# mindspore-lab/minddiffusion

Measured on AMD Instinct MI355X. Metric: 512x512 txt2img latents/sec (50-step DDIM), higher is better.
Workload: dtype f16; 1 GPU; SDv2 txt2img 512x512 (64x64 latent), 50-step DDIM, CFG 9.0, batch 1 per GPU (BASELINE.json configs[1]); synthetic seeded weights + synthetic text conditioning; global_batch=1, parallelism=batch-shard x1, hip_graph=True, rccl_world_size=1, broadcast_bytes=0, ddim_steps=50, unet_batch_per_gpu=2, sampler=ddim, cfg_dup_prefix=False

## Files before the change

include/mdx.h:

```cpp
#ifndef MDX_H_
#define MDX_H_

#include <stddef.h>
#include <stdint.h>

#ifdef __cplusplus
extern "C" {
#endif

#define MDX_OK 0
#define MDX_E_INVALID (-1)
#define MDX_E_WORKSPACE (-2)
#define MDX_E_HIP (-3)

typedef void* mdx_stream_t;

int mdx_version(void);
const char* mdx_last_error(void);
int mdx_set_option(const char* name, int value);
int mdx_get_option(const char* name, int* value);

int mdx_nchw_to_nhwc_f16(const float* x, void* y, int B, int C, int H, int W, int Cpad, mdx_stream_t s);
int mdx_nhwc_to_nchw_f32(const void* x, float* y, int B, int C, int H, int W, int Cstride, mdx_stream_t s);

// ... 77 lines not shown
    float xattn_scale;
    const float* act_slope;
    int act_slope_n;
    int geglu_unit;
} mdx_gemm_desc;

#define MDX_GEMM_WS_HEAD 16384
#define MDX_EPI_NONE 0
#define MDX_EPI_GEGLU 1
#define MDX_EPI_GELU 2
#define MDX_EPI_QUICKGELU 3
#define MDX_EPI_PRELU 4
#define MDX_OUT_ROWMAJOR 0
#define MDX_OUT_TRANSPOSED 1
#define MDX_OUT_D2S2 2

int mdx_gemm_f16(const mdx_gemm_desc* d, mdx_stream_t s);
int mdx_gemm_release_counters(void);
int mdx_gemm_release_workspace(const void* workspace);
int mdx_gemm_bind_counters(const void* workspace, void* counters);
size_t mdx_gemm_workspace_bytes(const mdx_gemm_desc* d);
int mdx_gemm_check(const mdx_gemm_desc* d);
int mdx_gemm_query(const mdx_gemm_desc* d, int* out7);
int mdx_gemm_tune(const mdx_gemm_desc* d, mdx_stream_t s, void* flush, size_t flush_bytes, int reps, int* best4, float* us2);

int mdx_groupnorm_from_splitk_f16(const mdx_gemm_desc* prod, const float* gamma, const float* beta, void* y, int groups,
                                  float eps, int silu, mdx_stream_t s);
int mdx_groupnorm_from_splitk_ok(const mdx_gemm_desc* prod, int groups);

int mdx_attention_f16(const void* q, long q_bs, int q_ld, const void* k, long k_bs, int k_ld, const void* vt,
                      long vt_bs, int vt_ld, void* o, long o_bs, int o_ld, int B, int heads, int D, int Nq, int Nk,
                      float scale, mdx_stream_t s);

size_t mdx_attention_ws_bytes(int B, int heads, int D, int Nq, int Nk);
int mdx_attention_splitkv_f16(const void* q, long q_bs, int q_ld, const void* k, long k_bs, int k_ld, const void* vt,
                              long vt_bs, int vt_ld, void* o, long o_bs, int o_ld, int B, int heads, int D, int Nq, int Nk,
                              float scale, int kv_splits, void* ws, size_t ws_bytes, mdx_stream_t s);

typedef struct mdx_st_tail_desc {
    const void* attn_out;
    const void* tok;
    const void* x_in;
    void* out;
    const void* ctx_k;
    const void* ctx_vt;
    const void* wstream;
// ... 141 lines not shown
```

minddiffusion_amd/_lib.py:

```python
import ctypes
import os

_HERE = os.path.dirname(os.path.abspath(__file__))
LIB_PATH = os.environ.get("MDX_LIBRARY") or os.path.join(_HERE, "libmdx.so")

c_void_p = ctypes.c_void_p
c_int = ctypes.c_int
c_long = ctypes.c_long
c_float = ctypes.c_float
c_size_t = ctypes.c_size_t


class MdxError(RuntimeError):
    pass


class GemmDesc(ctypes.Structure):
    _fields_ = [
        ("a", c_void_p), ("a2", c_void_p), ("c1", c_int), ("c2", c_int),
        ("w", c_void_p), ("bias", c_void_p), ("rowbias", c_void_p), ("rowbias_ld", c_int),
        ("residual", c_void_p), ("residual_ld", c_int),
        ("out", c_void_p), ("out_ld", c_int),
        ("B", c_int), ("H", c_int), ("W", c_int), ("N", c_int),
        ("ksize", c_int), ("stride", c_int), ("upsample", c_int),
# ... 58 lines not shown
                                  c_int, c_float, c_int, c_void_p, c_void_p]),
    "mdx_groupnorm_query": (c_int, [c_int, c_int, c_int, c_int, c_int, c_int, ctypes.POINTER(c_int)]),
    "mdx_groupnorm_colstats_f16": (c_int, [c_void_p, c_int, c_void_p, c_int, c_void_p, c_int, c_void_p, c_int, c_void_p,
                                           c_void_p, c_void_p, c_void_p, c_int, c_void_p, c_int, c_int, c_int, c_float,
                                           c_int, c_void_p]),
    "mdx_colstats_fold_f32": (c_int, [c_void_p, c_int, c_void_p, c_int, c_int, c_int, c_void_p]),
    "mdx_groupnorm_from_splitk_f16": (c_int, [ctypes.POINTER(GemmDesc), c_void_p, c_void_p, c_void_p, c_int, c_float, c_int,
                                              c_void_p]),
    "mdx_groupnorm_from_splitk_ok": (c_int, [ctypes.POINTER(GemmDesc), c_int]),
    "mdx_groupnorm_scaleshift_f16": (c_int, [c_void_p, c_int, c_void_p, c_int, c_void_p, c_void_p, c_void_p, c_void_p,
                                             c_int, c_void_p, c_int, c_int, c_int, c_float, c_int, c_void_p, c_void_p]),
    "mdx_layernorm_f16": (c_int, [c_void_p, c_void_p, c_void_p, c_void_p, c_int, c_int, c_float, c_void_p]),
    "mdx_gemm_f16": (c_int, [ctypes.POINTER(GemmDesc), c_void_p]),
    "mdx_gemm_workspace_bytes": (c_size_t, [ctypes.POINTER(GemmDesc)]),
    "mdx_gemm_release_workspace": (c_int, [c_void_p]),
    "mdx_gemm_bind_counters": (c_int, [c_void_p, c_void_p]),
    "mdx_st_tail_sched_barriers": (c_int, [c_int, c_int]),
    "mdx_st_head_sched_barriers": (c_int, [c_int, c_int]),
    "mdx_gemm_release_counters": (c_int, []),
    "mdx_gemm_tune": (c_int, [ctypes.POINTER(GemmDesc), c_void_p, c_void_p, c_size_t, c_int, ctypes.POINTER(c_int),
                              ctypes.POINTER(ctypes.c_float)]),
    "mdx_gemm_check": (c_int, [ctypes.POINTER(GemmDesc)]),
    "mdx_gemm_query": (c_int, [ctypes.POINTER(GemmDesc), ctypes.POINTER(c_int)]),
    "mdx_attention_f16": (c_int, [c_void_p, c_long, c_int, c_void_p, c_long, c_int, c_void_p, c_long, c_int,
                                  c_void_p, c_long, c_int, c_int, c_int, c_int, c_int, c_int, c_float, c_void_p]),
    "mdx_attention_ws_bytes": (c_size_t, [c_int, c_int, c_int, c_int, c_int]),
    "mdx_attention_splitkv_f16": (c_int, [c_void_p, c_long, c_int, c_void_p, c_long, c_int, c_void_p, c_long, c_int,
                                          c_void_p, c_long, c_int, c_int, c_int, c_int, c_int, c_int, c_float, c_int, c_void_p,
                                          c_size_t, c_void_p]),
    "mdx_attention_causal_f16": (c_int, [c_void_p, c_long, c_int, c_void_p, c_long, c_int, c_void_p, c_long, c_int,
                                  c_void_p, c_long, c_int, c_int, c_int, c_int, c_int, c_int, c_float, c_void_p]),
    "mdx_st_head_f16": (c_int, [ctypes.POINTER(StHeadDesc), c_void_p]),
    "mdx_st_head_supported": (c_int, [c_int, c_int, c_int]),
    "mdx_st_head_stream_bytes": (c_size_t, [c_int]),
    "mdx_st_tail_f16": (c_int, [ctypes.POINTER(StTailDesc), c_void_p]),
    "mdx_st_tail_supported": (c_int, [c_int, c_int, c_int, c_int, c_int]),
    "mdx_st_tail_stream_bytes": (c_size_t, [c_int]),
    "mdx_lora_merge_f16": (c_int, [ctypes.POINTER(LoraMergeDesc), c_void_p]),
    "mdx_timestep_embedding_f32": (c_int, [c_void_p, c_void_p, c_int, c_int, c_float, c_void_p]),
    "mdx_dense_small_f32": (c_int, [c_void_p, c_int, c_void_p, c_void_p, c_void_p, c_int, c_int, c_int, c_int,
                                    c_int, c_int, c_void_p]),
    "mdx_sampler_step_f32": (c_int, [c_void_p, c_void_p, c_void_p, c_int, c_float, c_void_p, c_void_p, c_void_p,
                                     c_void_p, c_float, c_float, c_float, c_float, c_float, c_void_p, c_void_p,
                                     c_void_p, c_void_p, c_int, c_int, c_int, c_int, c_void_p]),
    "mdx_sampler_step_pred_f32": (c_int, [c_void_p, c_void_p, c_void_p, c_void_p, c_int, c_float, c_int, c_float, c_float,
                                          c_void_p, c_void_p, c_void_p, c_void_p, c_float, c_float, c_float, c_float,
# ... 77 lines not shown
```

minddiffusion_amd/csrc/gemm.hip:

```cpp
#include "mdx_common.h"
#include "gemm_internal.h"

#include <algorithm>
#include <type_traits>

namespace {


template <int BM, int BN, int BK, int NS, bool SWAP, bool FASTK, int NW, bool GNA = false, bool EXT = false>
__global__ __launch_bounds__(NW * 64, NW == 4 ? 2 : 1) void gemm_kernel(const GemmParams p) {
    mdx_kernarg_touch<sizeof(GemmParams)>();
    constexpr int WROWS = BM / (NW / 2);
    constexpr int TM = WROWS / 32;
    constexpr int TN = BN / 64;
    static_assert(TM >= 1, "tile too short for this many waves");
    constexpr int ROWB = BK * 2;
    constexpr int CPRW = BK / 8;
    constexpr int RPI = 64 / CPRW;
    constexpr int RP256 = 256 / ROWB;
    constexpr int KS = BK / 16;
    constexpr int A_BYTES = BM * ROWB;
    constexpr int B_BYTES = BN * ROWB;
    constexpr int STAGE = A_BYTES + B_BYTES;
    constexpr int AJ = BM / RPI / NW;
// ... 314 lines not shown
                rdfrag(I1{}, ks + 1);
                __builtin_amdgcn_sched_barrier(0);
                mfmas(I0{});
                __builtin_amdgcn_sched_barrier(0);
                if (ks + 2 < KS) {
                    rdfrag(I0{}, ks + 2);
                    __builtin_amdgcn_sched_barrier(0);
                }
                mfmas(I1{});
                __builtin_amdgcn_sched_barrier(0);
            }
        }
        rd = (rd + 1 == NS) ? 0 : rd + 1;
        wr = (wr + 1 == NS) ? 0 : wr + 1;
    }

    __syncthreads();
    trace_mark(p, 3);
    if constexpr (SWAP) asm volatile("" ::"v"(touch_ln), "v"(touch_s));
    gemm_epilogue<BM, BN, SWAP, NW, LinearRows, 0, 0, EXT>(p, acc, smem, LinearRows{m0}, n0, split, bpre, tile_m, tile_id);
    trace_mark(p, 4);
}

template <int BM, int BN, int NSB, bool SWAP, int PW, bool BDIR = false, bool W4 = false>
__global__ __launch_bounds__(BM * 2, BM == 128 ? 2 : 1) void conv3x3_halo_kernel(const GemmParams p) {
    static_assert(PW == 16 || (PW == 8 && BM == 128), "patch width 16, or 8 with two-sample tiles");
    static_assert(!W4 || (BDIR && BM == 128 && BN == 128 && !SWAP), "W4: weight-streaming 128 x 128 tiles with slab output");
    constexpr int NW = BM / 32;
    constexpr int PH = BM / 16;
    constexpr int HWD = PW + 2;
    constexpr int WROWS = W4 ? BM : BM / (NW / 2);
    constexpr int TM = WROWS / 32;
    constexpr int TN = W4 ? 1 : BN / 64;
    constexpr int HROWS = PW == 16 ? (PH + 2) * 18 : (BM / 64) * 100;
    constexpr int HINST = (HROWS + 7) / 8;
    constexpr int HALO_BYTES = HINST * 1024;
    constexpr int HJ = (HINST + NW - 1) / NW;
    constexpr int B_BYTES = BN * 128;
    constexpr int BJ = BN / 8 / NW;
    static_assert(BJ >= 1, "weight tile too small for this many loader waves");
    extern __shared__ __attribute__((aligned(16))) char smem[];
    mdx_kernarg_touch<sizeof(GemmParams)>();

    const int tid = threadIdx.x;
    const int lane = tid & 63;
    const int wave = __builtin_amdgcn_readfirstlane(tid >> 6);
    const int wm = W4 ? 0 : wave >> 1, wn = W4 ? wave : wave & 1;
    const int hi = lane >> 5;
    const int l31 = lane & 31;
// ... 159 lines not shown
                for (int r = 0; r < 16; ++r) {
                    const int row = i * 32 + (r & 3) + 8 * (r >> 2) + 4 * hi;
                    int m;
                    if constexpr (PW == 16)
                        m = (pb * p.H + py0) * p.W + px0 + (row >> 4) * p.W + (row & 15);
                    else
                        m = tile_m * BM + row;
                    if (m < p.M && n < p.N) wsz[(size_t)m * p.N + n] = acc[i][0][r];
                }
            trace_mark(p, 4);
            return;
        } else {
            if constexpr (PW == 16)
                gemm_epilogue<BM, BN, SWAP, NW, PatchRows, 0, 2>(p, acc, smem, PatchRows{(pb * p.H + py0) * p.W + px0, p.W, pb}, n0,
                                                                          split, bpre, tile_m, tile_id);
            else
                gemm_epilogue<BM, BN, SWAP, NW>(p, acc, smem, LinearRows{tile_m * BM}, n0, split, bpre, tile_m, tile_id);
            trace_mark(p, 4);
            return;
        }
    }
    if constexpr (!BDIR) {
    float2* gn_tab = reinterpret_cast<float2*>(smem + 2 * HALO_BYTES + NSB * B_BYTES);
    if constexpr (PW == 16) {
        if (p.gn_cs) {
            float2* csum = reinterpret_cast<float2*>(smem);
            const int cpg = p.cin >> 5;
            const float2* src = reinterpret_cast<const float2*>(p.gn_cs) + (size_t)pb * p.gn_nrb * p.cin;
            for (int c = tid; c < p.cin; c += NW * 64) {
                float su = 0.f, sq = 0.f;
                int k = 0;
                for (; k + 8 <= p.gn_nrb; k += 8) {
                    float2 v[8];
#pragma unroll
                    for (int e = 0; e < 8; ++e) v[e] = src[(size_t)(k + e) * p.cin + c];
#pragma unroll
                    for (int e = 0; e < 8; ++e) {
                        su += v[e].x;
                        sq += v[e].y;
                    }
                }
                for (; k < p.gn_nrb; ++k) {
                    const float2 v = src[(size_t)k * p.cin + c];
                    su += v.x;
                    sq += v.y;
                }
                csum[c] = make_float2(su, sq);
// ... 14 lines not shown
                const float a = p.gn_gamma[c] * rsqrtf(var + p.gn_eps);
                gn_tab[c] = make_float2(a, p.gn_beta[c] - mean * a);
            }
            __syncthreads();
        }
    }
    auto gn_transform = [&](int chunk, int hb) {
#pragma unroll
        for (int q = 0; q < HJ; ++q) {
            if (wave * HJ + q >= HINST || hal_off[q] == MDX_OOB) continue;
            char* pc = smem + hb * HALO_BYTES + (wave * HJ + q) * 1024 + lane * 16;
            const int ch0 = chunk * 64 + (int)((hal_off[q] >> 4) & 7u) * 8;
            const f16x8 x = *reinterpret_cast<const f16x8*>(pc);
            f16x8 y;
#pragma unroll
            for (int e = 0; e < 8; ++e) {
                const float2 t = gn_tab[ch0 + e];
                const float v = (float)x[e] * t.x + t.y;
                y[e] = (f16)(p.gn_silu ? silu_f(v) : v);
            }
            *reinterpret_cast<f16x8*>(pc) = y;
        }
    };
#pragma unroll
    for (int q = 0; q < HJ; ++q) dma_halo(q, c_begin, 0);
#pragma unroll
    for (int i = 0; i < NSB - 1; ++i)
        if (i < nt) dma_b(kt_begin + i, i);

    int t = 0;
    int rd = 0, wr = NSB - 1;
    trace_mark(p, 1);
    for (int c = c_begin; c < c_end; ++c) {
        const int hb = (c - c_begin) & 1;
        const bool more = c + 1 < c_end;
#pragma unroll
        for (int tap = 0; tap < 9; ++tap, ++t) {
            if (NSB >= 4 && t + 2 < nt)
                asm volatile("s_waitcnt vmcnt(%0)" ::"n"(2 * BJ) : "memory");
            else if (NSB >= 3 && t + 1 < nt)
                asm volatile("s_waitcnt vmcnt(%0)" ::"n"(BJ) : "memory");
            else
                asm volatile("s_waitcnt vmcnt(0)" ::: "memory");
            if constexpr (PW == 16) {
                if (tap == 0 && p.gn_cs) {
                    gn_transform(c, hb);
// ... 50 lines not shown
                rdfrag(I0{}, 0); rdfrag(I1{}, 1); rdfrag(I2{}, 2); rdfrag(I3{}, 3);
                __builtin_amdgcn_sched_barrier(0);
                mfmas(I0{}); mfmas(I1{}); mfmas(I2{}); mfmas(I3{});
            } else {
                rdfrag(I0{}, 0);
                __builtin_amdgcn_sched_barrier(0);
#pragma unroll
                for (int ks = 0; ks < 4; ks += 2) {
                    rdfrag(I1{}, ks + 1);
                    __builtin_amdgcn_sched_barrier(0);
                    mfmas(I0{});
                    __builtin_amdgcn_sched_barrier(0);
                    if (ks + 2 < 4) {
                        rdfrag(I0{}, ks + 2);
                        __builtin_amdgcn_sched_barrier(0);
                    }
                    mfmas(I1{});
                    __builtin_amdgcn_sched_barrier(0);
                }
            }
            rd = (rd + 1 == NSB) ? 0 : rd + 1;
            wr = (wr + 1 == NSB) ? 0 : wr + 1;
        }
    }

    if (p.skip_w) {
        constexpr int SA_BYTES = BM * 128;
        static_assert(2 * SA_BYTES <= 2 * HALO_BYTES && NSB >= 2, "skip tiles reuse the halo / ring areas");
        const __amdgpu_buffer_rsrc_t rs_s1 = make_rsrc(p.skip_a, p.skip_a_bytes);
        const __amdgpu_buffer_rsrc_t rs_s2 = make_rsrc(p.skip_a2 ? p.skip_a2 : p.skip_a, p.skip_a2 ? p.skip_a2_bytes : p.skip_a_bytes);
        const __amdgpu_buffer_rsrc_t rs_sw = make_rsrc(p.skip_w, p.skip_w_bytes);
        const int sk_begin = split * p.skip_kt_per_split, sk_end = min(p.skip_kt, sk_begin + p.skip_kt_per_split);
        constexpr int SAJ = BM / 8 / NW;
        int s_pix[SAJ];
        unsigned s_cb[SAJ];
#pragma unroll
        for (int j = 0; j < SAJ; ++j) {
            const int row = (wave * SAJ + j) * 8 + lrow;
            int pix;
            if constexpr (PW == 16) {
                pix = (pb * p.H + py0 + (row >> 4)) * p.W + px0 + (row & 15);
            } else {
                pix = tile_m * BM + row;
                if (pix >= p.M) pix = -1;
            }
            s_pix[j] = pix;
// ... 304 lines not shown
            launch_one<BM, BN, BK, NS, false, false, NW>(p, grid, st);
    }
}

template <int BM, int BN>
bool launch_bn(const GemmParams& p, int ns, bool swap, bool fastk, dim3 grid, hipStream_t st, bool nw8 = false) {
    if constexpr (BM == 128) {
        if (nw8 && (ns == 2 || ns == 3)) {
            if (ns == 2) launch_cfg<128, BN, 64, 2, 8>(p, swap, fastk, grid, st); else launch_cfg<128, BN, 64, 3, 8>(p, swap, fastk, grid, st);
            return true;
        }
    }
    if (ns == 2) launch_cfg<BM, BN, 64, 2, 4>(p, swap, fastk, grid, st);
    else if (ns == 3) launch_cfg<BM, BN, 64, 3, 4>(p, swap, fastk, grid, st);
    else if (BM == 128 && ns == 4) launch_cfg<128, BN, 64, 4, 4>(p, swap, fastk, grid, st);
    else if (BM == 128 && ns == 5) launch_cfg<128, BN, 64, 5, 4>(p, swap, fastk, grid, st);
    else if (BM == 64 && ns == 4) launch_cfg<64, BN, 64, 4, 4>(p, swap, fastk, grid, st);
    else if (BM == 64 && ns == 5) launch_cfg<64, BN, 64, 5, 4>(p, swap, fastk, grid, st);
    else if (BM == 64 && ns == 6) launch_cfg<64, BN, 64, 6, 4>(p, swap, fastk, grid, st);
    else return false;
    return true;
}

template <int BM, int BN, int NSB, bool SWAP, int PW = 16, bool BDIR = false, bool W4 = false>
void launch_halo(const GemmParams& p, dim3 grid, hipStream_t st) {
    constexpr size_t hinst = ((PW == 16 ? (BM / 16 + 2) * 18 : (BM / 64) * 100) + 7) / 8;
    constexpr size_t ring = 2 * hinst * 1024 + (BDIR ? 0 : (size_t)NSB * BN * 128);
    constexpr size_t epi = (size_t)BM * (BN + 8) * 2 + 4096;
    constexpr size_t lds0 = ring > epi ? ring : epi;
    constexpr size_t gn_tab_max = (BDIR || PW != 16) ? 0 : 640 * 8;
    const size_t lds = lds0 + (p.gn_cs ? (size_t)p.cin * 8 : 0);
    static MdxPerDeviceOnce attr_once;
    if (attr_once.first()) {
        (void)hipFuncSetAttribute(reinterpret_cast<const void*>(&conv3x3_halo_kernel<BM, BN, NSB, SWAP, PW, BDIR, W4>),
                                  hipFuncAttributeMaxDynamicSharedMemorySize, (int)(lds0 + gn_tab_max));
    }
    hipLaunchKernelGGL((conv3x3_halo_kernel<BM, BN, NSB, SWAP, PW, BDIR, W4>), grid, dim3(BM * 2), lds, st, p);
}

template <int BN, int PW>
void launch_halo_bdir(const GemmParams& p, bool swap, dim3 grid, hipStream_t st) {
    if (swap) launch_halo<128, BN, 2, true, PW, true>(p, grid, st); else launch_halo<128, BN, 2, false, PW, true>(p, grid, st);
}
template <int PW>
void launch_halo_bdir_w4(const GemmParams& p, dim3 grid, hipStream_t st) {
    launch_halo<128, 128, 2, false, PW, true, true>(p, grid, st);
}

template <int BM, int BN, int PW = 16>
void launch_halo_cfg(const GemmParams& p, int nsb, bool swap, dim3 grid, hipStream_t st) {
    if (nsb == 4) {
        if (swap) launch_halo<BM, BN, 4, true, PW>(p, grid, st); else launch_halo<BM, BN, 4, false, PW>(p, grid, st);
    } else if (nsb == 3) {
        if (swap) launch_halo<BM, BN, 3, true, PW>(p, grid, st); else launch_halo<BM, BN, 3, false, PW>(p, grid, st);
    } else {
        if (swap) launch_halo<BM, BN, 2, true, PW>(p, grid, st); else launch_halo<BM, BN, 2, false, PW>(p, grid, st);
    }
}

}

int mdx_gemm_launch_plan(const GemmParams& p, const GemmPlan& pl, hipStream_t st) {
    const dim3 grid = pl.grid;
    const bool swap = pl.swap, wide = pl.bn == 128;
    int rc;
    switch (pl.form) {
        case GEMM_CONV8P:
            rc = mdx_conv8p_launch(p, pl.bn, st);
            if (rc != MDX_OK) return rc;
            MDX_LAUNCH_CHECK("mdx_gemm_f16(conv8p)");
            return MDX_OK;
        case GEMM_LEAN:
        case GEMM_LEAN_XA:
            rc = mdx_dense_launch(p, pl, st);
            if (rc != MDX_OK) return rc;
            break;
        case GEMM_HALO:
            if (pl.bm == 256) {
                if (wide) launch_halo_cfg<256, 128>(p, pl.ring, swap, grid, st); else launch_halo_cfg<256, 64>(p, pl.ring, swap, grid, st);
            } else if (pl.pw == 8) {
                if (wide) launch_halo_cfg<128, 128, 8>(p, pl.ring, swap, grid, st); else launch_halo_cfg<128, 64, 8>(p, pl.ring, swap, grid, st);
            } else {
                if (wide) launch_halo_cfg<128, 128>(p, pl.ring, swap, grid, st); else launch_halo_cfg<128, 64>(p, pl.ring, swap, grid, st);
            }
            break;
        case GEMM_HALO_FRAG:
            if (pl.pw == 8) {
                if (wide) launch_halo_bdir<128, 8>(p, swap, grid, st); else launch_halo_bdir<64, 8>(p, swap, grid, st);
            } else {
                if (wide) launch_halo_bdir<128, 16>(p, swap, grid, st); else launch_halo_bdir<64, 16>(p, swap, grid, st);
            }
            break;
        case GEMM_HALO_FRAG_W4:
            if (pl.pw == 8) launch_halo_bdir_w4<8>(p, grid, st); else launch_halo_bdir_w4<16>(p, grid, st);
            break;
        case GEMM_GNA:
            if (pl.bm == 64) {
                if (wide) launch_gna<64, 128>(p, pl.ring, swap, grid, st); else launch_gna<64, 64>(p, pl.ring, swap, grid, st);
            } else {
                if (wide) launch_gna<128, 128>(p, pl.ring, swap, grid, st); else launch_gna<128, 64>(p, pl.ring, swap, grid, st);
            }
            break;
        case GEMM_EXT:
            if (pl.bm == 64) {
                if (wide) launch_ext<64, 128>(p, pl.ring, swap, grid, st); else launch_ext<64, 64>(p, pl.ring, swap, grid, st);
            } else {
                if (wide) launch_ext<128, 128>(p, pl.ring, swap, grid, st); else launch_ext<128, 64>(p, pl.ring, swap, grid, st);
            }
// ... 31 lines not shown
```

minddiffusion_amd/csrc/gemm_internal.h:

```cpp
#pragma once
#include "mdx_common.h"

namespace mdx_int {

struct GemmParams {
    const f16* a;
    const f16* a2;
    const f16* w;
    const float* bias;
    const float* rowbias;
    const f16* residual;
    f16* out;
    f16* out2;
    float* ws;
    unsigned* tickets;
    int c1, c2, cin;
    int rowbias_ld, residual_ld, out_ld, out2_ld, n_split;
    float* stats_out;
    float* colstats_out;
    const float* ln_stats;
    const float* ln_s;
    int ln_nt;
    int bn_hint;
    int st_hint;
// ... 28 lines not shown
    unsigned inv_tiles_n, inv_tiles_m;
    unsigned res_bytes;
    const f16* xa_k;
    const f16* xa_vt;
    int xa_len, xa_cap;
    float xa_scale_log2;
    const float* act_slope;
    int act_slope_n;
    int d2s_c;
    int geglu_unit;
};

}
using mdx_int::GemmParams;

enum GemmForm {
    GEMM_GENERIC,
    GEMM_GENERIC_NW8,
    GEMM_GNA,
    GEMM_EXT,
    GEMM_LEAN,
    GEMM_LEAN_XA,
    GEMM_HALO,
    GEMM_HALO_FRAG,
    GEMM_HALO_FRAG_W4,
    GEMM_CONV8P
};
enum GemmReduce { GEMM_REDUCE_NONE, GEMM_REDUCE_PLAIN, GEMM_REDUCE_EXT, GEMM_REDUCE_COLSTATS, GEMM_REDUCE_DEFERRED };
struct TunedEntry;
struct GemmPlan {
    GemmForm form;
    int bm, bn;
    int ring;
    int pw;
    int nsplit;
    bool fixup;
    bool swap, fastk;
    dim3 grid;
    const TunedEntry* tuned;
    int colstats_rows;
    GemmReduce reduce;
    size_t ws_head, ws_per_split;
};
int mdx_gemm_launch_plan(const GemmParams& p, const GemmPlan& pl, hipStream_t st);

bool mdx_dense_takes_desc(const GemmParams& p, int bn);
// ... 663 lines not shown
```

minddiffusion_amd/csrc/gemm_plan.hip:

```cpp
#include "mdx_common.h"
#include "gemm_internal.h"

#include <stdlib.h>

#include <algorithm>
#include <map>
#include <mutex>
#include <utility>
#include <vector>

static int fill_params(const mdx_gemm_desc* d, GemmParams& p) {
    MDX_REQUIRE(d && d->a && d->w && d->out, "mdx_gemm_f16: null pointer");
    MDX_REQUIRE(d->ksize == 1 || d->ksize == 3, "mdx_gemm_f16: ksize must be 1 or 3 (got %d)", d->ksize);
    MDX_REQUIRE(d->stride == 1 || d->stride == 2, "mdx_gemm_f16: stride must be 1 or 2");
    MDX_REQUIRE(!(d->upsample && d->stride != 1), "mdx_gemm_f16: upsample requires stride 1");
    MDX_REQUIRE(d->B > 0 && d->H > 0 && d->W > 0 && d->N > 0, "mdx_gemm_f16: bad extents");
    MDX_REQUIRE(d->c1 > 0 && d->c1 % 8 == 0 && d->c2 >= 0 && d->c2 % 8 == 0, "mdx_gemm_f16: c1/c2 must be multiples of 8");
    MDX_REQUIRE((d->c2 == 0) == (d->a2 == nullptr), "mdx_gemm_f16: a2/c2 mismatch");
    MDX_REQUIRE(d->N % 8 == 0, "mdx_gemm_f16: N must be a multiple of 8 (got %d)", d->N);
    p.a = (const f16*)d->a;
    p.a2 = (const f16*)d->a2;
    p.w = (const f16*)d->w;
    p.bias = d->bias;
    p.rowbias = d->rowbias;
// ... 172 lines not shown
    const size_t ab = (size_t)d->B * d->H * d->W * d->c1 * 2, a2b = (size_t)d->B * d->H * d->W * d->c2 * 2;
    p.kt64 = (p.K + 63) / 64;
    const size_t wb = (size_t)((p.N + 63) / 64) * p.kt64 * 8192;
    MDX_REQUIRE(ab <= 0x80000000ull && a2b <= 0x80000000ull && wb <= 0x80000000ull,
                "mdx_gemm_f16: operand larger than 2 GiB is not addressable by one buffer descriptor");
    p.a_bytes = (unsigned)ab;
    p.a2_bytes = (unsigned)a2b;
    p.w_bytes = (unsigned)wb;
    return MDX_OK;
}

struct TunedEntry {
    int M, N, K, ksize, bm, bn, ns;
    int var1;
    int st;
};
static const TunedEntry g_tuned[] = {
#include "gemm_tuned.inc"
    {0, 0, 0, 0, 0, 0, 0, 0, 0}};
static const TunedEntry g_tuned160[] = {
#include "gemm_tuned160.inc"
    {0, 0, 0, 0, 0, 0, 0, 0, 0}};

static int tuned_variant(const GemmParams& p) {
    return (p.c2 > 0 ? 1 : 0) | (p.epilogue == MDX_EPI_PRELU ? 2048 : p.epilogue << 1) | (p.n_split ? 8 : 0) | (p.ln_stats ? 16 : 0) |
           (p.stats_out ? 32 : 0) |
           (p.out_mode == MDX_OUT_TRANSPOSED ? 64 : 0) | (p.colstats_out ? 128 : 0) | (p.residual ? 256 : 0) |
           (p.rowbias ? 512 : 0) | (p.d2s_c ? 1024 : 0);
}

static bool halo8_eligible(const GemmParams& p) {
    if (!mdx_opt(MDX_OPT_GEMM_HALO8)) return false;
    return p.H == 8 && p.W == 8;
}

static bool halo_epilogue_ok(const GemmParams& p) {
    return !p.d2s_c && (p.epilogue == MDX_EPI_NONE || p.epilogue == MDX_EPI_GEGLU);
}

static bool halo_eligible(const GemmParams& p, int bm) {
    if (!mdx_opt(MDX_OPT_GEMM_HALO)) return false;
    if (!halo_epilogue_ok(p)) return false;
    if (!(p.ksize == 3 && p.stride == 1 && !p.upsample && p.c2 == 0 && p.cin % 64 == 0 && p.out_mode == MDX_OUT_ROWMAJOR))
        return false;
    if (p.out_bs) return false;
    if (p.residual && (size_t)p.M * (size_t)p.residual_ld * 2 >= 0x80000000ull) return false;
    if (bm == 128 && halo8_eligible(p)) return true;
    return p.H % (bm / 16) == 0 && p.W % 16 == 0;
}

static const TunedEntry* lookup_tuned(const GemmParams& p) {
    const bool use_table = mdx_opt(MDX_OPT_GEMM_TUNED) && !mdx_opt(MDX_OPT_GEMM_BM) && !mdx_opt(MDX_OPT_GEMM_BN);
    if (!use_table || p.bn_hint || p.st_hint || p.stride != 1 || p.upsample) return nullptr;
    if (p.epilogue == MDX_EPI_PRELU || p.d2s_c) return nullptr;
    const int var1 = tuned_variant(p) + 1;
    if (mdx_dense_takes_desc(p, 160))
        for (const TunedEntry* e = g_tuned160; e->M; ++e)
            if (e->M == p.M && e->N == p.N && e->K == p.K && e->ksize == p.ksize && e->var1 == var1 && e->bn == 160) return e;
    const TunedEntry* any = nullptr;
    for (const TunedEntry* e = g_tuned; e->M; ++e)
        if (e->M == p.M && e->N == p.N && e->K == p.K && e->ksize == p.ksize) {
            if (e->var1 == var1) {
                any = e;
                break;
            }
            if (e->var1 == 0 && !any) any = e;
        }
    if (!any) return nullptr;
    if (any->bm == 256 && !halo_eligible(p, 256)) return nullptr;
    return (any->bm >= 128 || !halo_eligible(p, 128)) ? any : nullptr;
}

static void cost_model_tiling(const GemmParams& p, int bn, int forced_ns, int forced_bm, int& best_bm, int& best_ns) {
    const int envbm = mdx_opt(MDX_OPT_GEMM_BM);
    const int kt = (p.K + 63) / 64;
    const int chunks = p.cin / 64;
    const double slab_mb = (double)p.M * p.N * 4.0 / 1048576.0;
    const double unique_mb = ((double)p.N * p.K + (double)p.M * p.cin) * 2.0 / 1048576.0;
    best_bm = 128, best_ns = 1;
    double best_cost = 1e30;
    static const int order[3] = {128, 256, 64};
// ... 67 lines not shown
    p.bk = 64;
    p.ktiles = (p.K + 63) / 64;
    p.tickets = nullptr;
    auto colstats_rows = [&](bool halo) {
        if (p.out_mode != MDX_OUT_ROWMAJOR || p.epilogue != MDX_EPI_NONE || p.n_split || p.ln_stats || p.stats_out || p.out_bs ||
            p.d2s_c)
            return 0;
        if (pl.nsplit > 1 && !pl.fixup) return p.HoWo % CS_ROWS == 0 ? CS_ROWS : 0;
        if (halo) return pl.pw == 8 ? 0 : pl.bm;
        return p.HoWo % pl.bm == 0 ? pl.bm : 0;
    };
    if (conv8p_wanted(d, p)) {
        pl.form = GEMM_CONV8P;
        pl.bm = 256;
        pl.bn = mdx_conv8p_pick_bn(p, d->tile_n);
        pl.nsplit = 1;
        p.ktiles_per_split = p.ktiles;
        p.skip_kt_per_split = p.skip_w ? p.skip_kt : 0;
        pl.ws_head = mdx_conv8p_plan(p, pl.bn, sizing ? 0 : d->workspace_bytes, !sizing && d->workspace != nullptr, sizing);
        pl.colstats_rows = colstats_rows(true);
        return MDX_OK;
    }

    const TunedEntry* row = lookup_tuned(p);
    const int optbn = mdx_opt(MDX_OPT_GEMM_BN);
    int bn;
    if (p.epilogue == MDX_EPI_GEGLU) bn = (p.bn_hint == 160 || (row && row->bn == 160)) ? 160 : 128;
    else if (p.bn_hint == 64 || p.bn_hint == 128 || p.bn_hint == 160) bn = p.bn_hint;
    else if (row && row->bn) bn = row->bn;
    else if (optbn == 64 || optbn == 128) bn = optbn;
    else if (p.N % 128 == 0) bn = 128;
    else if (p.N % 64 == 0 || p.N < 128) bn = 64;
    else bn = (p.N % 128 > 64) ? 128 : 64;
    pl.tuned = (d->splitk <= 0 && d->tile_m <= 0) ? row : nullptr;
    const int stages = pl.tuned ? pl.tuned->st : p.st_hint;
    int bm, ns;
    if (pl.tuned) bm = row->bm, ns = row->ns;
    else cost_model_tiling(p, bn, d->splitk, d->tile_m, bm, ns);
    pl.bm = bm;
    pl.bn = bn;
    if (ns > 1) {
        pl.ws_per_split = std::max(split_bytes(d, p, bm, bn, 2, &pl.ws_head), split_bytes(d, p, bm, bn, 1 << 30, &pl.ws_head));
    }
    if (sizing) {
        pl.nsplit = ns;
        return MDX_OK;
    }
// ... 38 lines not shown
    ns = p.nsplit = pl.nsplit = (p.ktiles + p.ktiles_per_split - 1) / p.ktiles_per_split;
    p.skip_kt_per_split = p.skip_w ? (p.skip_kt + ns - 1) / ns : 0;
    pl.fixup = ns > 1 && fixup_eligible(d, p, bm, bn, ns);
    if (ns <= 1) pl.ws_head = pl.ws_per_split = 0;
    if (pl.fixup) p.tickets = reinterpret_cast<unsigned*>(p.ws);
    else if (ns > 1) p.ws += MDX_TICKET_SLOTS;
    if (ns > 1 && !pl.fixup)
        pl.reduce = d->defer_reduce ? GEMM_REDUCE_DEFERRED : p.colstats_out ? GEMM_REDUCE_COLSTATS
                    : (p.epilogue == MDX_EPI_PRELU || p.d2s_c) ? GEMM_REDUCE_EXT : GEMM_REDUCE_PLAIN;
    pl.colstats_rows = colstats_rows(halo);

    p.tiles_m = (p.M + bm - 1) / bm;
    p.tiles_n = (p.N + bn - 1) / bn;
    pl.fastk = (p.cin % 64 == 0) && (p.c2 == 0 || p.c1 % 64 == 0);
    MDX_REQUIRE(pl.fastk || p.c2 == 0, "mdx_gemm_f16: two-source input needs c1 %% 64 == 0 and Cin %% 64 == 0");
    const int ntiles = p.tiles_m * p.tiles_n;
    p.tiles_per_xcd = (ntiles + 7) / 8;
    p.inv_tiles_n = p.tiles_n > 1 ? (unsigned)((0x100000000ull + (unsigned)p.tiles_n - 1) / (unsigned)p.tiles_n) : 0u;
    p.inv_tiles_m = p.tiles_m > 1 ? (unsigned)((0x100000000ull + (unsigned)p.tiles_m - 1) / (unsigned)p.tiles_m) : 0u;
    p.res_bytes = p.residual ? (unsigned)std::min<size_t>((size_t)p.M * (size_t)p.residual_ld * 2, 0x7fffffffull) : 0u;
    p.n_fastest = ((size_t)p.M * p.cin >= (size_t)p.N * p.K) ? 1 : 0;
    p.spread = (p.tiles_m == 1 && mdx_opt(MDX_OPT_GEMM_SPREAD)) ? 1 : 0;
    pl.grid = p.spread ? dim3(ntiles * ns, 1) : dim3(8 * p.tiles_per_xcd, ns);
    const bool nw8 = stages >= 10;
    const int st_req = nw8 ? stages - 8 : stages;
    const int optring = mdx_opt(MDX_OPT_GEMM_RING);
    int ring = optring;
    if (!(optring >= 2 && optring <= 5)) {
        ring = (ntiles * ns <= 256 || bm + bn <= 192) ? 3 : 2;
        if (st_req >= 2 && st_req <= 6) ring = st_req;
    }
    pl.swap = (ns == 1 || pl.fixup) && (p.out_mode == MDX_OUT_ROWMAJOR);
    const bool lean = !halo && mdx_dense_takes(p, bm, bn, ring, ns, pl.fixup, nw8);
    MDX_REQUIRE(bn != 160 || lean, "mdx_gemm_f16: the 128 x 160 tile exists in the lean dense kernel only (ring depth 2 | 3, four waves; got stages %d)",
                stages);

    MDX_REQUIRE(!d->defer_reduce || ns > 1, "mdx_gemm_f16: defer_reduce set but the launch does not split K");
    MDX_REQUIRE(!p.xa_k || (lean && bn == 64 && ns == 1 && (p.HoWo % bm) == 0),
                "mdx_gemm_f16: the cross-attention epilogue needs the lean dense kernel on %d x 64 tiles inside one sample (got tile %d x %d, %d splits)",
                bm, bm, bn, ns);
    MDX_REQUIRE(!d->w_frag || halo, "mdx_gemm_f16: fragment-major weights (w_frag) are read by the HALO 3x3 conv only");

    if (halo) {
        if (d->w_frag) {
            MDX_REQUIRE(bm == 128, "mdx_gemm_f16: fragment-major weights run on 128-row HALO tiles only (got tile_m %d)", bm);
            pl.form = (bn == 128 && ns > 1 && !pl.fixup) ? GEMM_HALO_FRAG_W4 : GEMM_HALO_FRAG;
        } else {
            pl.form = GEMM_HALO;
            pl.ring = (bm == 256 || bn == 64) ? 3 : 2;
            if (st_req >= 2 && st_req <= 4) pl.ring = st_req;
            if (mdx_opt(MDX_OPT_HALO_NSB) >= 2 && mdx_opt(MDX_OPT_HALO_NSB) <= 4) pl.ring = mdx_opt(MDX_OPT_HALO_NSB);
        }
    } else if (p.gn_cs || p.epilogue == MDX_EPI_PRELU || p.d2s_c) {
        pl.form = p.gn_cs ? GEMM_GNA : GEMM_EXT;
        pl.ring = ring >= 3 ? 3 : 2;
    } else if (lean) {
        pl.form = p.xa_k ? GEMM_LEAN_XA : GEMM_LEAN;
        pl.ring = ring;
    } else {
        pl.form = (nw8 && bm == 128 && (ring == 2 || ring == 3)) ? GEMM_GENERIC_NW8 : GEMM_GENERIC;
        pl.ring = ring;
        MDX_REQUIRE(ring <= (bm == 128 ? 5 : 6), "mdx_gemm_f16: unsupported tile configuration bk=%d ns=%d", 64,
                    (optring >= 2 && optring <= 5) ? optring : 2);
    }
    return MDX_OK;
}
// ... 140 lines not shown
    return pl.ws_head + (pl.nsplit > 1 ? (size_t)pl.nsplit * pl.ws_per_split : 0);
}

extern "C" int mdx_gemm_check(const mdx_gemm_desc* d) {
    GemmParams p{};
    GemmPlan pl;
    const int rc = fill_params(d, p);
    if (rc != MDX_OK) return rc;
    MDX_REQUIRE(p.c2 == 0 || (p.cin % 64 == 0 && p.c1 % 64 == 0), "mdx_gemm_f16: two-source input needs c1 %% 64 == 0 and Cin %% 64 == 0");
    return plan_gemm(d, p, pl);
}

extern "C" int mdx_gemm_query(const mdx_gemm_desc* d, int* out7) {
    GemmParams p{};
    GemmPlan pl;
    int rc = fill_params(d, p);
    if (rc != MDX_OK) return rc;
    MDX_REQUIRE(out7, "mdx_gemm_query: null output");
    rc = plan_gemm(d, p, pl);
    if (rc != MDX_OK) return rc;
    out7[0] = pl.bm;
    out7[1] = pl.bn;
    out7[2] = pl.nsplit;
    const bool conv = pl.form == GEMM_HALO || pl.form == GEMM_HALO_FRAG || pl.form == GEMM_HALO_FRAG_W4 || pl.form == GEMM_CONV8P;
    out7[3] = conv ? 1 : (pl.form == GEMM_LEAN || pl.form == GEMM_LEAN_XA) ? 2 : 0;
    out7[4] = (pl.tuned && pl.bn != 160) ? 1 : 0;
    out7[5] = pl.colstats_rows;
    out7[6] = pl.fixup ? 1 : 0;
    return MDX_OK;
}

int mdx_internal_split_info(const mdx_gemm_desc* d, MdxSplitInfo* info) {
    GemmParams p{};
    GemmPlan pl;
    int rc = fill_params(d, p);
    if (rc != MDX_OK) return rc;
    rc = plan_gemm(d, p, pl);
    if (rc != MDX_OK) return rc;
    MDX_REQUIRE(p.out_mode == MDX_OUT_ROWMAJOR && p.epilogue == MDX_EPI_NONE && !p.n_split && !p.ln_stats && !p.stats_out &&
                    !p.out_bs && !p.colstats_out && p.out_ld == p.N && p.N % 8 == 0,
                "deferred split-K reduce: plain dense row-major producers only");
    info->ws = p.ws;
    info->nsplit = pl.nsplit;
    info->M = p.M;
    info->N = p.N;
    info->HoWo = p.HoWo;
    info->B = p.B;
    info->bias = p.bias;
    info->rowbias = p.rowbias;
    info->rowbias_ld = p.rowbias_ld;
    info->residual = p.residual;
// ... 114 lines not shown
```

minddiffusion_amd/ops.py:

```python
import ctypes
import os

import torch

from . import _lib
from ._lib import GemmDesc, EPI_NONE, EPI_GEGLU, EPI_GELU, EPI_QUICKGELU, OUT_ROWMAJOR, OUT_TRANSPOSED
from ._lib import EPI_PRELU, OUT_D2S2

f16 = torch.float16
f32 = torch.float32


_OPTIONS = {"unet_st_tail": int(os.environ.get("MDX_UNET_ST_TAIL", "-1")),
            "unet_st_head": int(os.environ.get("MDX_UNET_ST_HEAD", "-1")),
            "unet_conv_stream": int(os.environ.get("MDX_UNET_CONV_STREAM", "128")),
            "gn_colstats_fold": int(os.environ.get("MDX_GN_COLSTATS_FOLD", "0")),
            "unet_gn_splitk_fuse": int(os.environ.get("MDX_UNET_GN_SPLITK_FUSE", "256")),
            "unet_conv_stream_w4": int(os.environ.get("MDX_UNET_CONV_STREAM_W4", "0")),
            "unet_skip_fuse": int(os.environ.get("MDX_UNET_SKIP_FUSE", "1")),
            "unet_gn_conv_fuse": int(os.environ.get("MDX_UNET_GN_CONV_FUSE", "0")),
            "unet_tune_first_use": int(os.environ.get("MDX_UNET_TUNE_FIRST_USE", "0")),
            "unet_subpixel_upsample": int(os.environ.get("MDX_UNET_SUBPIXEL_UPSAMPLE", "1")),
            "unet_gn_proj_fuse": int(os.environ.get("MDX_UNET_GN_PROJ_FUSE", "0")),
            "unet_xattn_fuse": int(os.environ.get("MDX_UNET_XATTN_FUSE", "1")),
# ... 392 lines not shown


def new_gemm_workspace(nbytes, device):
    import weakref
    base = torch.zeros((_WS_HEAD + max(int(nbytes), 16)) // 4 + 1, dtype=f32, device=device)
    ws = base[_WS_HEAD // 4:]
    lib = _lib.load()
    _lib.check(lib.mdx_gemm_bind_counters(ctypes.c_void_p(ws.data_ptr()), ctypes.c_void_p(base.data_ptr())),
               "mdx_gemm_bind_counters")
    weakref.finalize(ws, lib.mdx_gemm_release_workspace, ctypes.c_void_p(ws.data_ptr()))
    return ws


def gemm_check(desc):
    return _lib.load().mdx_gemm_check(ctypes.byref(desc)) == 0


def gemm_query(desc):
    out = (ctypes.c_int * 7)()
    _lib.check(_lib.load().mdx_gemm_query(ctypes.byref(desc), out), "mdx_gemm_query")
    return tuple(int(v) for v in out)


tune_cache = {}
_tune_flush = {}


def gemm_shape_key(d):
    var = ((1 if d.c2 > 0 else 0) | (d.epilogue << 1) | (8 if d.n_split else 0) | (16 if d.ln_stats else 0)
           | (32 if d.stats_out else 0) | (64 if d.out_mode == 1 else 0) | (128 if d.colstats_out else 0)
           | (256 if d.residual else 0) | (512 if d.rowbias else 0) | (1024 if d.skip_w else 0) | (2048 if d.gn_gamma else 0)
           | (4096 if d.w_sub else 0))
    return (d.B * d.H * d.W, d.N, d.ksize * d.ksize * (d.c1 + d.c2), d.ksize, d.stride, d.upsample, var, d.B, d.H, d.W)


def gemm_tune(desc, reps=5, cold=True):
    flush, nbytes = None, 0
    if cold:
        dev = torch.cuda.current_device()
        if dev not in _tune_flush:
            _tune_flush[dev] = torch.empty(512 << 20, dtype=torch.uint8, device=f"cuda:{dev}")
        flush, nbytes = ctypes.c_void_p(_tune_flush[dev].data_ptr()), _tune_flush[dev].numel()
    best, us = (ctypes.c_int * 4)(), (ctypes.c_float * 2)()
    _lib.check(_lib.load().mdx_gemm_tune(ctypes.byref(desc), _stream(), flush, nbytes, int(reps), best, us), "mdx_gemm_tune")
    return tuple(int(v) for v in best) + (float(us[0]), float(us[1]))

# ... 401 lines not shown
```

Measured before the change: 5.376 latents/s.

## Add row-stage HALO 3x3 conv variant staging three weight taps per ring slot

After: 5.366 latents/s. Within noise of the previous version (-0.2%).

```diff
diff --git a/include/mdx.h b/include/mdx.h
--- a/include/mdx.h
+++ b/include/mdx.h
@@ -123,6 +123,7 @@
 size_t mdx_gemm_workspace_bytes(const mdx_gemm_desc* d);
 int mdx_gemm_check(const mdx_gemm_desc* d);
 int mdx_gemm_query(const mdx_gemm_desc* d, int* out7);
+int mdx_gemm_query_form(const mdx_gemm_desc* d, int* out2);
 int mdx_gemm_tune(const mdx_gemm_desc* d, mdx_stream_t s, void* flush, size_t flush_bytes, int reps, int* best4, float* us2);
 
 int mdx_groupnorm_from_splitk_f16(const mdx_gemm_desc* prod, const float* gamma, const float* beta, void* y, int groups,
diff --git a/minddiffusion_amd/_lib.py b/minddiffusion_amd/_lib.py
--- a/minddiffusion_amd/_lib.py
+++ b/minddiffusion_amd/_lib.py
@@ -104,6 +104,7 @@
                               ctypes.POINTER(ctypes.c_float)]),
     "mdx_gemm_check": (c_int, [ctypes.POINTER(GemmDesc)]),
     "mdx_gemm_query": (c_int, [ctypes.POINTER(GemmDesc), ctypes.POINTER(c_int)]),
+    "mdx_gemm_query_form": (c_int, [ctypes.POINTER(GemmDesc), ctypes.POINTER(c_int)]),
     "mdx_attention_f16": (c_int, [c_void_p, c_long, c_int, c_void_p, c_long, c_int, c_void_p, c_long, c_int,
                                   c_void_p, c_long, c_int, c_int, c_int, c_int, c_int, c_int, c_float, c_void_p]),
     "mdx_attention_ws_bytes": (c_size_t, [c_int, c_int, c_int, c_int, c_int]),
diff --git a/minddiffusion_amd/csrc/gemm.hip b/minddiffusion_amd/csrc/gemm.hip
--- a/minddiffusion_amd/csrc/gemm.hip
+++ b/minddiffusion_amd/csrc/gemm.hip
@@ -360,9 +360,10 @@
     trace_mark(p, 4);
 }
 
-template <int BM, int BN, int NSB, bool SWAP, int PW, bool BDIR = false, bool W4 = false>
-__global__ __launch_bounds__(BM * 2, BM == 128 ? 2 : 1) void conv3x3_halo_kernel(const GemmParams p) {
+template <int BM, int BN, int NSB, bool SWAP, int PW, bool BDIR = false, bool W4 = false, int TPS = 1>
+__global__ __launch_bounds__(BM * 2, (BM == 128 && TPS == 1) ? 2 : 1) void conv3x3_halo_kernel(const GemmParams p) {
     static_assert(PW == 16 || (PW == 8 && BM == 128), "patch width 16, or 8 with two-sample tiles");
+    static_assert(TPS == 1 || (TPS == 3 && PW == 16 && !BDIR && (NSB == 2 || NSB == 3)), "row stages: 8 x 16 / 16 x 16 patches, LDS weight ring of 2 | 3");
     static_assert(!W4 || (BDIR && BM == 128 && BN == 128 && !SWAP), "W4: weight-streaming 128 x 128 tiles with slab output");
     constexpr int NW = BM / 32;
     constexpr int PH = BM / 16;
@@ -568,7 +569,7 @@
     }
     if constexpr (!BDIR) {
     float2* gn_tab = reinterpret_cast<float2*>(smem + 2 * HALO_BYTES + NSB * B_BYTES);
-    if constexpr (PW == 16) {
+    if constexpr (PW == 16 && TPS == 1) {
         if (p.gn_cs) {
             float2* csum = reinterpret_cast<float2*>(smem);
             const int cpg = p.cin >> 5;
@@ -629,6 +630,93 @@
             *reinterpret_cast<f16x8*>(pc) = y;
         }
     };
+    if constexpr (TPS == 3) {
+        static_assert(HJ == 6, "two halo slices per stage, three stages per chunk");
+        constexpr int ST_BYTES = 3 * B_BYTES;
+        auto dma_b3 = [&](int kt0, int slot) {
+            char* sb = smem + 2 * HALO_BYTES + slot * ST_BYTES;
+#pragma unroll
+            for (int u = 0; u < 3; ++u)
+#pragma unroll
+                for (int j = 0; j < BJ; ++j)
+                    dma16s(rs_w, sb + u * B_BYTES + (wave * BJ + j) * 1024, b_off[j], (unsigned)(kt0 + u) * 8192u);
+        };
+        const int nst = nt / 3;
+#pragma unroll
+        for (int q = 0; q < HJ; ++q) dma_halo(q, c_begin, 0);
+#pragma unroll
+        for (int i = 0; i < NSB - 1; ++i) dma_b3(kt_begin + 3 * i, i);
+        int s = 0;
+        int rd = 0, wr = NSB - 1;
+        trace_mark(p, 1);
+        for (int c = c_begin; c < c_end; ++c) {
+            const int hb = (c - c_begin) & 1;
+            const bool more = c + 1 < c_end;
+#pragma unroll
+            for (int r = 0; r < 3; ++r, ++s) {
+                if (NSB == 3 && s + 1 < nst)
+                    asm volatile("s_waitcnt vmcnt(%0)" ::"n"(3 * BJ) : "memory");
+                else
+                    asm volatile("s_waitcnt vmcnt(0)" ::: "memory");
+                __builtin_amdgcn_s_barrier();
+                if (s == 0) trace_mark(p, 2);
+                if (more) {
+                    dma_halo(2 * r, c + 1, hb ^ 1);
+                    dma_halo(2 * r + 1, c + 1, hb ^ 1);
+                }
+                if (s + NSB - 1 < nst) dma_b3(kt_begin + 3 * (s + NSB - 1), wr);
+                __builtin_amdgcn_sched_barrier(0);
+                const char* sb = smem + rd * ST_BYTES;
+                f16x8 af[2][4][TM], bf[2][4][TN];
+                auto rdtap = [&](auto set_c, auto u_c) {
+                    constexpr int set = decltype(set_c)::value, u = decltype(u_c)::value;
+                    const int dq = r * HWD + u;
+                    const int a_key = ((((l31 & 15) + u) >> 1) & 7) << 4;
+#pragma unroll
+                    for (int ks = 0; ks < 4; ++ks) {
+#pragma unroll
+                        for (int i = 0; i < TM; ++i)
+                            af[set][ks][i] = *reinterpret_cast<const f16x8*>(smem + hb * HALO_BYTES + (hp0[i] + dq) * 128 + (((2 * ks + hi) << 4) ^ a_key));
+#pragma unroll
+                        for (int j = 0; j < TN; ++j)
+                            bf[set][ks][j] = *reinterpret_cast<const f16x8*>(sb + u * B_BYTES + b_row_off + j * 32 * 128 + (((2 * ks + hi) ^ swz_b) << 4));
+                    }
+                };
+                auto mfmatap = [&](auto set_c) {
+                    constexpr int set = decltype(set_c)::value;
+#pragma unroll
+                    for (int ks = 0; ks < 4; ++ks)
+#pragma unroll
+                        for (int i = 0; i < TM; ++i)
+#pragma unroll
+                            for (int j = 0; j < TN; ++j) {
+                                if constexpr (SWAP)
+                                    acc[i][j] = __builtin_amdgcn_mfma_f32_32x32x16_f16(bf[set][ks][j], af[set][ks][i], acc[i][j], 0, 0, 0);
+                                else
+                                    acc[i][j] = __builtin_amdgcn_mfma_f32_32x32x16_f16(af[set][ks][i], bf[set][ks][j], acc[i][j], 0, 0, 0);
+                            }
+                };
+                using I0 = std::integral_constant<int, 0>;
+                using I1 = std::integral_constant<int, 1>;
+                using I2 = std::integral_constant<int, 2>;
+                rdtap(I0{}, I0{});
+                __builtin_amdgcn_sched_barrier(0);
+                rdtap(I1{}, I1{});
+                __builtin_amdgcn_sched_barrier(0);
+                mfmatap(I0{});
+                __builtin_amdgcn_sched_barrier(0);
+                rdtap(I0{}, I2{});
+                __builtin_amdgcn_sched_barrier(0);
+                mfmatap(I1{});
+                __builtin_amdgcn_sched_barrier(0);
+                mfmatap(I0{});
+                __builtin_amdgcn_sched_barrier(0);
+                rd = (rd + 1 == NSB) ? 0 : rd + 1;
+                wr = (wr + 1 == NSB) ? 0 : wr + 1;
+            }
+        }
+    }
+    if constexpr (TPS == 1) {
 #pragma unroll
     for (int q = 0; q < HJ; ++q) dma_halo(q, c_begin, 0);
 #pragma unroll
@@ -725,6 +813,7 @@
             rd = (rd + 1 == NSB) ? 0 : rd + 1;
             wr = (wr + 1 == NSB) ? 0 : wr + 1;
         }
+    }
     }
 
     if (p.skip_w) {
@@ -1075,20 +1164,21 @@
     return true;
 }
 
-template <int BM, int BN, int NSB, bool SWAP, int PW = 16, bool BDIR = false, bool W4 = false>
+template <int BM, int BN, int NSB, bool SWAP, int PW = 16, bool BDIR = false, bool W4 = false, int TPS = 1>
 void launch_halo(const GemmParams& p, dim3 grid, hipStream_t st) {
     constexpr size_t hinst = ((PW == 16 ? (BM / 16 + 2) * 18 : (BM / 64) * 100) + 7) / 8;
-    constexpr size_t ring = 2 * hinst * 1024 + (BDIR ? 0 : (size_t)NSB * BN * 128);
+    constexpr size_t ring = 2 * hinst * 1024 + (BDIR ? 0 : (size_t)NSB * TPS * BN * 128);
     constexpr size_t epi = (size_t)BM * (BN + 8) * 2 + 4096;
     constexpr size_t lds0 = ring > epi ? ring : epi;
-    constexpr size_t gn_tab_max = (BDIR || PW != 16) ? 0 : 640 * 8;
+    static_assert(lds0 <= 160 * 1024, "more LDS than a CU has");
+    constexpr size_t gn_tab_max = (BDIR || PW != 16 || TPS != 1) ? 0 : 640 * 8;
     const size_t lds = lds0 + (p.gn_cs ? (size_t)p.cin * 8 : 0);
     static MdxPerDeviceOnce attr_once;
     if (attr_once.first()) {
-        (void)hipFuncSetAttribute(reinterpret_cast<const void*>(&conv3x3_halo_kernel<BM, BN, NSB, SWAP, PW, BDIR, W4>),
+        (void)hipFuncSetAttribute(reinterpret_cast<const void*>(&conv3x3_halo_kernel<BM, BN, NSB, SWAP, PW, BDIR, W4, TPS>),
                                   hipFuncAttributeMaxDynamicSharedMemorySize, (int)(lds0 + gn_tab_max));
     }
-    hipLaunchKernelGGL((conv3x3_halo_kernel<BM, BN, NSB, SWAP, PW, BDIR, W4>), grid, dim3(BM * 2), lds, st, p);
+    hipLaunchKernelGGL((conv3x3_halo_kernel<BM, BN, NSB, SWAP, PW, BDIR, W4, TPS>), grid, dim3(BM * 2), lds, st, p);
 }
 
 template <int BN, int PW>
@@ -1109,6 +1199,21 @@
     } else {
         if (swap) launch_halo<BM, BN, 2, true, PW>(p, grid, st); else launch_halo<BM, BN, 2, false, PW>(p, grid, st);
     }
+}
+
+template <int BM, int BN>
+bool launch_halo_row(const GemmParams& p, int nsb, bool swap, dim3 grid, hipStream_t st) {
+    if (nsb == 2) {
+        if (swap) launch_halo<BM, BN, 2, true, 16, false, false, 3>(p, grid, st); else launch_halo<BM, BN, 2, false, 16, false, false, 3>(p, grid, st);
+        return true;
+    }
+    if constexpr (BN == 64) {
+        if (nsb == 3) {
+            if (swap) launch_halo<BM, 64, 3, true, 16, false, false, 3>(p, grid, st); else launch_halo<BM, 64, 3, false, 16, false, false, 3>(p, grid, st);
+            return true;
+        }
+    }
+    return false;
 }
 
 }
@@ -1137,6 +1242,14 @@
                 if (wide) launch_halo_cfg<128, 128>(p, pl.ring, swap, grid, st); else launch_halo_cfg<128, 64>(p, pl.ring, swap, grid, st);
             }
             break;
+        case GEMM_HALO_ROW: {
+            bool ok = false;
+            if (pl.bm == 256 && !wide) ok = launch_halo_row<256, 64>(p, pl.ring, swap, grid, st);
+            else if (pl.bm == 128) ok = wide ? launch_halo_row<128, 128>(p, pl.ring, swap, grid, st) : launch_halo_row<128, 64>(p, pl.ring, swap, grid, st);
+            MDX_REQUIRE(ok, "mdx_gemm_f16: internal error: the plan names a row-stage HALO tile %d x %d at ring depth %d that is not built", pl.bm,
+                        pl.bn, pl.ring);
+            break;
+        }
         case GEMM_HALO_FRAG:
             if (pl.pw == 8) {
                 if (wide) launch_halo_bdir<128, 8>(p, swap, grid, st); else launch_halo_bdir<64, 8>(p, swap, grid, st);
diff --git a/minddiffusion_amd/csrc/gemm_internal.h b/minddiffusion_amd/csrc/gemm_internal.h
--- a/minddiffusion_amd/csrc/gemm_internal.h
+++ b/minddiffusion_amd/csrc/gemm_internal.h
@@ -74,6 +74,7 @@
     GEMM_LEAN,
     GEMM_LEAN_XA,
     GEMM_HALO,
+    GEMM_HALO_ROW,
     GEMM_HALO_FRAG,
     GEMM_HALO_FRAG_W4,
     GEMM_CONV8P
diff --git a/minddiffusion_amd/csrc/gemm_plan.hip b/minddiffusion_amd/csrc/gemm_plan.hip
--- a/minddiffusion_amd/csrc/gemm_plan.hip
+++ b/minddiffusion_amd/csrc/gemm_plan.hip
@@ -218,6 +218,10 @@
 #include "gemm_tuned160.inc"
     {0, 0, 0, 0, 0, 0, 0, 0, 0}};
 
+static const TunedEntry g_tuned_row[] = {
+#include "gemm_tuned_row.inc"
+    {0, 0, 0, 0, 0, 0, 0, 0, 0}};
+
 static int tuned_variant(const GemmParams& p) {
     return (p.c2 > 0 ? 1 : 0) | (p.epilogue == MDX_EPI_PRELU ? 2048 : p.epilogue << 1) | (p.n_split ? 8 : 0) | (p.ln_stats ? 16 : 0) |
            (p.stats_out ? 32 : 0) |
@@ -245,7 +249,7 @@
     return p.H % (bm / 16) == 0 && p.W % 16 == 0;
 }
 
-static const TunedEntry* lookup_tuned(const GemmParams& p) {
+static const TunedEntry* lookup_tuned(const GemmParams& p, bool w_frag) {
     const bool use_table = mdx_opt(MDX_OPT_GEMM_TUNED) && !mdx_opt(MDX_OPT_GEMM_BM) && !mdx_opt(MDX_OPT_GEMM_BN);
     if (!use_table || p.bn_hint || p.st_hint || p.stride != 1 || p.upsample) return nullptr;
     if (p.epilogue == MDX_EPI_PRELU || p.d2s_c) return nullptr;
@@ -253,6 +257,11 @@
     if (mdx_dense_takes_desc(p, 160))
         for (const TunedEntry* e = g_tuned160; e->M; ++e)
             if (e->M == p.M && e->N == p.N && e->K == p.K && e->ksize == p.ksize && e->var1 == var1 && e->bn == 160) return e;
+    if (!p.gn_cs && !w_frag && !halo8_eligible(p))
+        for (const TunedEntry* e = g_tuned_row; e->M; ++e)
+            if (e->M == p.M && e->N == p.N && e->K == p.K && e->ksize == p.ksize && e->var1 == var1 && (e->st == 12 || e->st == 13) &&
+                halo_eligible(p, e->bm))
+                return e;
     const TunedEntry* any = nullptr;
     for (const TunedEntry* e = g_tuned; e->M; ++e)
         if (e->M == p.M && e->N == p.N && e->K == p.K && e->ksize == p.ksize) {
@@ -366,7 +375,7 @@
         return MDX_OK;
     }
 
-    const TunedEntry* row = lookup_tuned(p);
+    const TunedEntry* row = lookup_tuned(p, d->w_frag != 0);
     const int optbn = mdx_opt(MDX_OPT_GEMM_BN);
     int bn;
     if (p.epilogue == MDX_EPI_GEGLU) bn = (p.bn_hint == 160 || (row && row->bn == 160)) ? 160 : 128;
@@ -451,8 +460,9 @@
     p.n_fastest = ((size_t)p.M * p.cin >= (size_t)p.N * p.K) ? 1 : 0;
     p.spread = (p.tiles_m == 1 && mdx_opt(MDX_OPT_GEMM_SPREAD)) ? 1 : 0;
     pl.grid = p.spread ? dim3(ntiles * ns, 1) : dim3(8 * p.tiles_per_xcd, ns);
-    const bool nw8 = stages >= 10;
-    const int st_req = nw8 ? stages - 8 : stages;
+    const bool nw8 = stages == 10 || stages == 11;
+    const bool rowst = stages == 12 || stages == 13;
+    const int st_req = nw8 ? stages - 8 : rowst ? 0 : stages;
     const int optring = mdx_opt(MDX_OPT_GEMM_RING);
     int ring = optring;
     if (!(optring >= 2 && optring <= 5)) {
@@ -470,7 +480,22 @@
                 bm, bm, bn, ns);
     MDX_REQUIRE(!d->w_frag || halo, "mdx_gemm_f16: fragment-major weights (w_frag) are read by the HALO 3x3 conv only");
 
-    if (halo) {
+    if (rowst) {
+        MDX_REQUIRE(halo && pl.pw == 16,
+                    "mdx_gemm_f16: stages = %d (row-stage HALO form) needs a launch that resolves to the HALO 3x3 conv on 8 x 16 / 16 x 16 "
+                    "patches (3x3, stride 1, single source, Cin %% 64 == 0, H %% 8 == 0, W %% 16 == 0; not the two-sample tiles of 8 x 8 images)",
+                    stages);
+        MDX_REQUIRE(!d->w_frag, "mdx_gemm_f16: stages = %d (row-stage HALO form) reads tile-major weights through the LDS ring, not w_frag", stages);
+        MDX_REQUIRE(!p.gn_cs, "mdx_gemm_f16: stages = %d (row-stage HALO form) does not carry the fused input GroupNorm (gn_colstats)", stages);
+        MDX_REQUIRE(!(bm == 256 && bn == 128), "mdx_gemm_f16: stages = %d (row-stage HALO form): a 256 x 128 tile does not fit the LDS of a CU", stages);
+        MDX_REQUIRE(!(bn == 128 && stages == 13),
+                    "mdx_gemm_f16: stages = 13 (row-stage HALO form, ring depth 3) with 128-column tiles does not fit the LDS of a CU (use 12)");
+    }
+
+    if (halo && rowst) {
+        pl.form = GEMM_HALO_ROW;
+        pl.ring = stages - 10;
+    } else if (halo) {
         if (d->w_frag) {
             MDX_REQUIRE(bm == 128, "mdx_gemm_f16: fragment-major weights run on 128-row HALO tiles only (got tile_m %d)", bm);
             pl.form = (bn == 128 && ns > 1 && !pl.fixup) ? GEMM_HALO_FRAG_W4 : GEMM_HALO_FRAG;
@@ -657,11 +682,38 @@
     out7[0] = pl.bm;
     out7[1] = pl.bn;
     out7[2] = pl.nsplit;
-    const bool conv = pl.form == GEMM_HALO || pl.form == GEMM_HALO_FRAG || pl.form == GEMM_HALO_FRAG_W4 || pl.form == GEMM_CONV8P;
+    const bool conv = pl.form == GEMM_HALO || pl.form == GEMM_HALO_ROW || pl.form == GEMM_HALO_FRAG || pl.form == GEMM_HALO_FRAG_W4 || pl.form == GEMM_CONV8P;
     out7[3] = conv ? 1 : (pl.form == GEMM_LEAN || pl.form == GEMM_LEAN_XA) ? 2 : 0;
-    out7[4] = (pl.tuned && pl.bn != 160) ? 1 : 0;
+    out7[4] = (pl.tuned && pl.bn != 160 && pl.form != GEMM_HALO_ROW) ? 1 : 0;
     out7[5] = pl.colstats_rows;
     out7[6] = pl.fixup ? 1 : 0;
+    return MDX_OK;
+}
+
+extern "C" int mdx_gemm_query_form(const mdx_gemm_desc* d, int* out2) {
+    GemmParams p{};
+    GemmPlan pl;
+    int rc = fill_params(d, p);
+    if (rc != MDX_OK) return rc;
+    MDX_REQUIRE(out2, "mdx_gemm_query_form: null output");
+    rc = plan_gemm(d, p, pl);
+    if (rc != MDX_OK) return rc;
+    int f = 0;
+    switch (pl.form) {
+        case GEMM_GENERIC: f = 0; break;
+        case GEMM_GENERIC_NW8: f = 1; break;
+        case GEMM_GNA: f = 2; break;
+        case GEMM_EXT: f = 3; break;
+        case GEMM_LEAN: f = 4; break;
+        case GEMM_LEAN_XA: f = 5; break;
+        case GEMM_HALO: f = 6; break;
+        case GEMM_HALO_FRAG: f = 7; break;
+        case GEMM_HALO_FRAG_W4: f = 8; break;
+        case GEMM_CONV8P: f = 9; break;
+        case GEMM_HALO_ROW: f = 10; break;
+    }
+    out2[0] = f;
+    out2[1] = pl.ring;
     return MDX_OK;
 }
 
diff --git a/minddiffusion_amd/csrc/gemm_tuned_row.inc b/minddiffusion_amd/csrc/gemm_tuned_row.inc
--- /dev/null
+++ b/minddiffusion_amd/csrc/gemm_tuned_row.inc
@@ -0,0 +1,3 @@
+    {512, 1280, 11520, 3, 128, 64, 3, 1, 13},
+    {512, 1280, 11520, 3, 128, 64, 3, 257, 13},
+    {512, 1280, 11520, 3, 128, 64, 3, 513, 13},
diff --git a/minddiffusion_amd/ops.py b/minddiffusion_amd/ops.py
--- a/minddiffusion_amd/ops.py
+++ b/minddiffusion_amd/ops.py
@@ -438,6 +438,15 @@
     return tuple(int(v) for v in out)
 
 
+FORM_HALO, FORM_HALO_ROW = 6, 10
+
+
+def gemm_query_form(desc):
+    out = (ctypes.c_int * 2)()
+    _lib.check(_lib.load().mdx_gemm_query_form(ctypes.byref(desc), out), "mdx_gemm_query_form")
+    return int(out[0]), int(out[1])
+
+
 tune_cache = {}
 _tune_flush = {}
 
```
